# hkust-vgd/pointwise

Hardware: AMD Instinct MI355X
Metric: conv3p fwd+bwd Mpoints/s (higher is better)
Workload: dtype f32; 1 GPU; cfg2 ModelNet40-shaped: B=32 clouds/GPU x N=2048, pointcnn2_acsd conv3p stack 3->9 s1, 9->9 s2, 9->9 s3, 9->9 s4 (+SELU), forward+backward, a different batch every step, next batch's neighbour search enqueued on a side stream under the current backward; global_batch=32, points_per_cloud=2048, parallelism=dp1, backward_kernel_choice=hint from Conv3pStack.tune() at set-up: short lists

## Files before the change

### include/conv3p.h

```cpp
#ifndef CONV3P_H
#define CONV3P_H

#include <stddef.h>
#include <stdint.h>

#ifdef __cplusplus
extern "C" {
#endif

#define CONV3P_ABI_VERSION 5

#define CONV3P_OK 0
#define CONV3P_ERR_INVALID_ARGUMENT 1
#define CONV3P_ERR_WORKSPACE 2
#define CONV3P_ERR_UNSUPPORTED 3
#define CONV3P_ERR_LAUNCH 4
#define CONV3P_ERR_NO_DEVICE 5

#define CONV3P_PASS_FORWARD 0
#define CONV3P_PASS_BACKWARD 1
#define CONV3P_PASS_NEIGHBOR_COUNT 2

size_t conv3p_workspace_bytes(int pass, int elem_bytes, int B, int N, int Cin, int Cout, int fz,
                              int fy, int fx);
// ... 284 lines not shown
                        size_t workspace_bytes, void *stream);

size_t conv3p_seg_head_weighted_workspace_bytes(size_t rows, int num_class);
int conv3p_seg_weight_total_f32(const int32_t *labels, size_t rows, int num_class, const float *class_weight,
                                const float *point_weight, double *total, void *workspace, size_t workspace_bytes,
                                void *stream);
int conv3p_seg_weight_total_f64(const int32_t *labels, size_t rows, int num_class, const double *class_weight,
                                const double *point_weight, double *total, void *workspace, size_t workspace_bytes,
                                void *stream);
int conv3p_seg_head_weighted_f32(const float *act, const int32_t *labels, size_t rows, int num_class,
                                 const float *class_weight, const float *point_weight, double label_smoothing,
                                 float grad_scale, const double *denominator, float *grad_act, int32_t *pred,
                                 double *loss_sum, int64_t *counts, void *workspace, size_t workspace_bytes, void *stream);
int conv3p_seg_head_weighted_f64(const double *act, const int32_t *labels, size_t rows, int num_class,
                                 const double *class_weight, const double *point_weight, double label_smoothing,
                                 double grad_scale, const double *denominator, double *grad_act, int32_t *pred,
                                 double *loss_sum, int64_t *counts, void *workspace, size_t workspace_bytes, void *stream);
size_t conv3p_seg_confusion_workspace_bytes(size_t rows, int num_class);
int conv3p_seg_confusion(const int32_t *labels, const int32_t *pred, size_t rows, int num_class, int64_t *confusion,
                         void *workspace, size_t workspace_bytes, void *stream);

#define CONV3P_OPT_MAX_TENSORS 16
int conv3p_momentum_step_f32(int n_tensors, float *const *params, const float *const *grads, float *const *accums,
                             const size_t *numels, float lr, float momentum, void *stream);
int conv3p_momentum_step_f64(int n_tensors, double *const *params, const double *const *grads, double *const *accums,
                             const size_t *numels, double lr, double momentum, void *stream);
int conv3p_fc_backward_step_f32(const float *x, float *W, float *b, const float *y, const float *dy, int M, int K, int N,
                                int act, float *dx, float *accum_W, float *accum_b, float lr, float momentum,
                                void *workspace, size_t workspace_bytes, void *stream);

size_t conv3p_grad_norm_workspace_bytes(void);
int conv3p_grad_norm_f32(int n_tensors, const float *const *grads, const size_t *numels, double *stats, int accumulate,
                         void *workspace, size_t workspace_bytes, void *stream);
int conv3p_grad_norm_f64(int n_tensors, const double *const *grads, const size_t *numels, double *stats, int accumulate,
                         void *workspace, size_t workspace_bytes, void *stream);
int conv3p_momentum_step_guarded_f32(int n_tensors, float *const *params, const float *const *grads, float *const *accums,
                                     const size_t *numels, float lr, float momentum, int nesterov, float clip_norm,
                                     int skip_nonfinite, const double *stats, void *stream);
int conv3p_momentum_step_guarded_f64(int n_tensors, double *const *params, const double *const *grads,
                                     double *const *accums, const size_t *numels, double lr, double momentum, int nesterov,
                                     double clip_norm, int skip_nonfinite, const double *stats, void *stream);

size_t conv3p_cls_tail_workspace_bytes(int M, int H, int C);
int conv3p_cls_tail_f32(const float *fc1, const float *W2, const float *b2, const int32_t *labels, int M, int H, int C,
                        int training, double rate, const float *keep_mask, uint64_t seed, uint64_t step, float grad_scale,
                        float *logits, int32_t *pred, float *dfc1, float *dW2, float *db2, uint8_t *keep_out,
                        double *loss_sum, int64_t *counts, void *workspace, size_t workspace_bytes, void *stream);
int conv3p_cls_tail_step_f32(const float *fc1, float *W2, float *b2, const int32_t *labels, int M, int H, int C,
                             int training, double rate, const float *keep_mask, uint64_t seed, uint64_t step,
                             float grad_scale, float *logits, int32_t *pred, float *dfc1, float *accum_W2, float *accum_b2,
                             float lr, float momentum, uint8_t *keep_out, double *loss_sum, int64_t *counts,
                             void *workspace, size_t workspace_bytes, void *stream);

int conv3p_profile_enable(int on);
int conv3p_profile_reset(void);
int conv3p_profile_kinds(void);
const char *conv3p_profile_name(int kind);
int conv3p_profile_read(int kind, uint64_t *launches, double *total_ms);

const char *conv3p_status_string(int status);
int conv3p_abi_version(void);

#ifdef __cplusplus
}
#endif
#endif
```

### pointwise_amd/_lib.py

```python
import ctypes
import os

_HERE = os.path.dirname(os.path.abspath(__file__))
LIB_PATH = os.environ.get("CONV3P_HIP_LIB") or os.path.join(_HERE, "csrc", "libconv3p_hip.so")

OK = 0
ERR_INVALID_ARGUMENT = 1
ERR_WORKSPACE = 2
ERR_UNSUPPORTED = 3
ERR_LAUNCH = 4
ERR_NO_DEVICE = 5

PASS_FORWARD = 0
PASS_BACKWARD = 1
PASS_NEIGHBOR_COUNT = 2
CACHE_POINTS_UNCHANGED = 1
CACHE_SPARSE_NEIGHBOURHOODS = 2
CACHE_DENSE_NEIGHBOURHOODS = 8
CACHE_PREPARE_DEEP_ORDERS = 4
CACHE_FUSED_FORWARD = 16
CACHE_FUSED_BACKWARD = 32
CACHE_FUSED_STACK = CACHE_FUSED_FORWARD | CACHE_FUSED_BACKWARD
CACHE_MATMUL_BF16 = 64
ABI_VERSION = 5
# ... 93 lines not shown
                                       ctypes.c_double, ctypes.c_double, ctypes.c_uint64, ctypes.c_uint64, _vp, _vp, _vp,
                                       _vp, _vp, _vp, _vp, _vp, _vp, _vp, _sz, _vp]),
    "conv3p_sort_order_workspace_bytes": (_sz, [_i, _i, _i]),
    "conv3p_sort_order_f32": (_i, [_vp, _i, _i, _i, _i, _vp, _vp, _sz, _vp]),
    "conv3p_provider_wide_workspace_bytes": (_sz, [_i, _i, _i]),
    "conv3p_scene_blocks_workspace_bytes": (_sz, [ctypes.c_int64, _i, _i, ctypes.c_float, ctypes.c_float]),
    "conv3p_scene_blocks_f32": (_i, [_vp, _vp, ctypes.c_int64, _i, _i, ctypes.c_float, ctypes.c_float, _i, _i, _i,
                                     ctypes.c_uint64, ctypes.c_uint64, _vp, _vp, _vp, _vp, _vp, _vp, _vp, _sz, _vp]),
    "conv3p_scene_vote": (_i, [_vp, _vp, _sz, ctypes.c_int64, _i, _vp, _vp]),
    "conv3p_scene_vote_labels_workspace_bytes": (_sz, [ctypes.c_int64, _i]),
    "conv3p_scene_vote_labels": (_i, [_vp, ctypes.c_int64, _i, _vp, _vp, _vp, _sz, _vp]),
    "conv3p_scene_blocks_cover_workspace_bytes": (_sz, [ctypes.c_int64, _i, _i, ctypes.c_float, ctypes.c_float]),
    "conv3p_scene_blocks_cover_f32": (_i, [_vp, _vp, ctypes.c_int64, _i, _i, ctypes.c_float, ctypes.c_float, _i, _i, _i,
                                           ctypes.c_uint64, ctypes.c_uint64, _vp, _vp, _vp, _vp, _vp, _vp, _vp, _sz, _vp]),
    "conv3p_scene_blocks_rooms_workspace_bytes": (_sz, [ctypes.c_int64, ctypes.c_int64, _i, _i, ctypes.c_float,
                                                        ctypes.c_float, _i]),
    "conv3p_scene_blocks_rooms_f32": (_i, [_vp, _vp, _vp, ctypes.c_int64, ctypes.c_int64, _i, _i, ctypes.c_float,
                                           ctypes.c_float, _i, _i, _i, _i, ctypes.c_uint64, ctypes.c_uint64, _vp, _vp, _vp,
                                           _vp, _vp, _vp, _vp, _vp, _vp, _vp, _sz, _vp]),
    "conv3p_scene_vote_scores_f32": (_i, [_vp, _vp, _sz, ctypes.c_int64, _i, _vp, _vp, _vp]),
    "conv3p_scene_score_labels_workspace_bytes": (_sz, [ctypes.c_int64, _i]),
    "conv3p_scene_score_labels": (_i, [_vp, ctypes.c_int64, _i, _vp, _vp, _vp, _sz, _vp]),
    "conv3p_grid_subsample_workspace_bytes": (_sz, [ctypes.c_int64, _i]),
    "conv3p_grid_subsample_f32": (_i, [_vp, _vp, ctypes.c_int64, _i, _i, ctypes.c_float, _i, _i, _i, _vp, _vp, _vp, _vp, _vp,
                                       _vp, _vp, _vp, _sz, _vp]),
    "conv3p_grid_project_labels": (_i, [_vp, _vp, ctypes.c_int64, ctypes.c_int64, _vp, _vp]),
    "conv3p_grid_subsample_rooms_workspace_bytes": (_sz, [ctypes.c_int64, ctypes.c_int64, _i]),
    "conv3p_grid_subsample_rooms_f32": (_i, [_vp, _vp, _vp, ctypes.c_int64, ctypes.c_int64, _i, _i, ctypes.c_float, _i, _i, _i,
                                             _vp, _vp, _vp, _vp, _vp, _vp, _vp, _vp, _vp, _vp, _vp, _sz, _vp]),
    "conv3p_grid_neighbors": (_i, [_vp, _vp, _vp, _vp, _i, ctypes.c_int64, _vp, _vp]),
    "conv3p_grid_interpolate_f32": (_i, [_vp, ctypes.c_int64, _i, _vp, _vp, _i, _vp, _vp, ctypes.c_int64, _i, _vp, _i, _vp,
                                         _vp, _vp, _vp]),
    "conv3p_grid_interpolate_i64": (_i, [_vp, ctypes.c_int64, _i, _vp, _vp, _i, _vp, _vp, ctypes.c_int64, _i, _vp, _i, _vp,
                                         _vp, _vp, _vp]),
    "conv3p_grid_interpolate_rings_workspace_bytes": (_sz, [ctypes.c_int64]),
    "conv3p_grid_interpolate_rings_f32": (_i, [_vp, ctypes.c_int64, _i, _vp, _vp, _i, _vp, _vp, _vp, _vp, ctypes.c_int64, _vp,
                                               _vp, ctypes.c_int64, _i, _vp, _i, _i, _vp, _vp, _vp, _vp, _vp, _vp, _sz, _vp]),
    "conv3p_grid_interpolate_rings_i64": (_i, [_vp, ctypes.c_int64, _i, _vp, _vp, _i, _vp, _vp, _vp, _vp, ctypes.c_int64, _vp,
                                               _vp, ctypes.c_int64, _i, _vp, _i, _i, _vp, _vp, _vp, _vp, _vp, _vp, _sz, _vp]),
    "conv3p_grid_normals_f32": (_i, [_vp, _i, _vp, _vp, _vp, _vp, ctypes.c_int64, ctypes.c_int64, _i, _vp, _vp, _vp, _vp, _vp,
                                     _vp, _vp]),
    "conv3p_grid_segments_workspace_bytes": (_sz, [ctypes.c_int64]),
    "conv3p_grid_segments": (_i, [_vp, _vp, ctypes.c_int64, _vp, _vp, ctypes.c_int64, _i, _i, _vp, _vp, _vp, _vp, _vp, _vp, _vp,
                                  _sz, _vp]),
    "conv3p_grid_absorb_workspace_bytes": (_sz, [ctypes.c_int64]),
    "conv3p_grid_absorb_segments": (_i, [_vp, _vp, ctypes.c_int64, _vp, _vp, _vp, _vp, _vp, ctypes.c_int64, _i, _i, _i, _i, _vp,
                                         _vp, _vp, _vp, _sz, _vp]),
    "conv3p_stack_scratch_bytes": (_sz, [ctypes.POINTER(StackDesc), _i, _i, _i]),
    "conv3p_workspace_bytes": (_sz, [_i] * 9),
    "conv3p_cache_bytes": (_sz, [_i, _i, _i, ctypes.POINTER(CacheConfig)]),
    "conv3p_cache_forget": (_i, [_vp]),
    "conv3p_cache_init": (_i, [_vp, _sz, _vp]),
    "conv3p_cache_fused_status": (_i, [_vp, ctypes.POINTER(ctypes.c_uint), ctypes.POINTER(ctypes.c_uint), ctypes.POINTER(ctypes.c_uint)]),
    "conv3p_profile_enable": (_i, [_i]),
    "conv3p_profile_reset": (_i, []),
    "conv3p_profile_kinds": (_i, []),
    "conv3p_profile_name": (ctypes.c_char_p, [_i]),
    "conv3p_profile_read": (_i, [_i, ctypes.POINTER(ctypes.c_uint64), ctypes.POINTER(ctypes.c_double)]),
    "conv3p_status_string": (ctypes.c_char_p, [_i]),
    "conv3p_abi_version": (_i, []),
}
for _sfx, _real in (("f32", ctypes.c_float), ("f64", ctypes.c_double)):
    for _name, _s in _sig(_real).items():
        SYMBOLS["conv3p_%s_%s" % (_name, _sfx)] = _s

SYMBOLS["conv3p_provider_batch_wide_f32"] = SYMBOLS["conv3p_provider_batch_f32"]

_LIB = None


class Conv3pLibraryError(RuntimeError):
    pass


def load():
    global _LIB
    if _LIB is not None:
        return _LIB
    if not os.path.exists(LIB_PATH):
        raise Conv3pLibraryError(
            "libconv3p_hip.so not found at %s -- run `python -m pointwise_amd.build` "
            "(there is no CPU fallback in the product path)" % LIB_PATH)
    lib = ctypes.CDLL(LIB_PATH)
    for name, (res, args) in SYMBOLS.items():
        try:
            fn = getattr(lib, name)
        except AttributeError:
            raise Conv3pLibraryError("libconv3p_hip.so does not export %s" % name)
        fn.restype = res
        fn.argtypes = args
    if lib.conv3p_abi_version() != ABI_VERSION:
        raise Conv3pLibraryError("libconv3p_hip.so ABI version mismatch")
    _LIB = lib
    return lib


def status_string(code):
    return load().conv3p_status_string(code).decode()
```

### pointwise_amd/csrc/conv3p_abi.hip

```cpp
#include "../../include/conv3p.h"
#include "conv3p_kernels.hpp"
#include "conv3p_stack_fused.hpp"
#include "conv3p_prestep.hpp"
#include "conv3p_head.hpp"
#include "conv3p_seg_head.hpp"
#include "conv3p_seg_head_weighted.hpp"
#include "conv3p_optim.hpp"
#include "conv3p_optim_guarded.hpp"
#include "conv3p_cls_tail.hpp"
#include "conv3p_provider.hpp"
#include "conv3p_sort_wide.hpp"
#include "conv3p_scene.hpp"
#include "conv3p_scene_cover.hpp"
#include "conv3p_scene_rooms.hpp"
#include "conv3p_grid.hpp"
#include "conv3p_grid_rooms.hpp"
#include "conv3p_grid_interp.hpp"
#include "conv3p_grid_interp_rings.hpp"
#include "conv3p_grid_normals.hpp"
#include "conv3p_grid_segments.hpp"

#include <hip/hip_runtime.h>
#include <algorithm>
#include <cmath>
#include <cstdio>
#include <cstdlib>
#include <cstring>
#include <map>
#include <mutex>
#include <vector>

using namespace conv3p;

namespace {

constexpr size_t kAlign = 256;
inline size_t up(size_t x) { return (x + kAlign - 1) / kAlign * kAlign; }

enum Kind { K_PREP = 0, K_SEARCH, K_FORWARD, K_BACKWARD, K_REDUCE, K_SELU, K_SELU_GRAD, K_MEMSET,
            K_DEEP_GEMM, K_DEEP_DW, K_TRANSPOSE, K_DEEP_ORDER, K_FC_FWD, K_FC_DX, K_FC_DW, K_DEEP_GEMM_BF16, K_DEEP_DW_BF16,
            K_GENERIC_FWD, K_GENERIC_BWD,
            K_SEG_HEAD,
            K_NKINDS };
const char *const kKindName[K_NKINDS] = {"prep_kernel", "search_kernel", "forward_kernel",
                                         "backward_kernel", "reduce_partials_kernel", "selu_kernel",
                                         "selu_grad_kernel", "memset", "deep_gemm_kernel", "deep_dw_kernel",
                                         "transpose_filter_kernel", "deep_order_kernel", "fc_forward_kernel",
                                         "fc_dx_kernel", "fc_dw_kernel", "deep_gemm_bf16_kernel", "deep_dw_bf16_kernel",
                                         "generic_forward_kernel", "generic_backward_kernel", "seg_head_kernel"};
struct Prof {
    std::mutex mu;
    bool on = false;
    struct Rec { int kind; hipEvent_t a, b; };
    std::vector<Rec> recs;
    std::vector<hipEvent_t> pool;
    hipEvent_t get()
    {
        if (!pool.empty()) { hipEvent_t e = pool.back(); pool.pop_back(); return e; }
        hipEvent_t e = nullptr;
        (void)hipEventCreate(&e);
        return e;
    }
} g_prof;

struct Scope {
    hipStream_t s;
    hipEvent_t b = nullptr;
    bool on;
    Scope(int kind, hipStream_t stream) : s(stream)
    {
        std::lock_guard<std::mutex> lk(g_prof.mu);
        on = g_prof.on;
        if (!on) return;
        hipEvent_t a = g_prof.get();
        b = g_prof.get();
        (void)hipEventRecord(a, s);
// ... 359 lines not shown
    return hip_ok();
}

template <typename SlotT> inline const uint32_t *sched_of(const SlotT &S)
{
#ifdef CONV3P_DEV_NO_SCHED
    return nullptr;
#else
    return S.sched;
#endif
}

constexpr unsigned long long kShortListsPerPoint = 35, kShortListsPerPointFused = 48;
template <typename T> bool fused_ok(const Call<T> &c);
template <typename T> SchedJob make_sched_job(const Call<T> &c, int slot, bool fused)
{
    const auto &S = c.L.slot[slot];
    return SchedJob{S.segs, S.sched, S.cursor, S.regime,
                    (fused ? kShortListsPerPointFused : kShortListsPerPoint) * (unsigned long long)c.d.B * (unsigned long long)c.d.N};
}

#ifndef CONV3P_DEV_FUSED_M
#define CONV3P_DEV_FUSED_M 6
#endif
template <typename T> bool fused_ok(const Call<T> &c)
{
#ifdef CONV3P_DEV_NO_FUSED_SEARCH
    return false;
#endif
    const Stencil<T> &st = c.st;
    if (c.L.ftab == nullptr || st.window) return false;
    for (int a = 0; a < 3; ++a)
        if (st.ext[a] > kFMaxExt) return false;
    return true;
}
template <typename T> FusedJob<T> make_fused_job(const Call<T> &c)
{
    const auto &S = c.L.slot[c.slot];
    FusedJob<T> j;
    j.st = c.st;
    j.cc = c.cc;
    j.count = S.count;
    j.tcount = S.tcount;
    j.pairs = S.pairs;
    j.segs = S.segs;
    j.qsegs = S.qsegs;
    j.qbm = S.qbm;
    j.qbm_hi = S.qbm_hi;
    for (int a = 0; a < 3; ++a)
        for (int k = 0; k < kFMaxExt; ++k)
            j.clo[a][k] = (float)(((double)k * c.st.step[a] - (double)c.st.full[a] * 0.5) * (double)kFR);
    return j;
}
inline int fused_mask_depth(int elem, int ntiles, int ntap_max, int maxfull_max)
{
    const int mmax = (ntiles + kWavesPerBlock - 1) / kWavesPerBlock;
    int M = std::min(mmax, (int)CONV3P_DEV_FUSED_M);
    if (ntiles <= 32) M = 1;
    if (M < 1) M = 1;
    while (M > 1 && fused_lds(ntap_max, maxfull_max, elem, M).total > 40 * 1024) --M;
    return fused_lds(ntap_max, maxfull_max, elem, M).total > kMaxLds ? 0 : M;
}
template <typename T> int launch_fused(const Call<T> &c, const FusedJobs<T> &jobs, const SchedJobs &sjobs, int njobs, bool schedule = true)
{
    const Dims &d = c.d;
    const BlockMap bm = make_blockmap(d);
    int ntap_max = 1, maxfull_max = 1;
    for (int k = 0; k < njobs; ++k) {
        ntap_max = std::max(ntap_max, jobs.job[k].st.ntap);
        maxfull_max = std::max(maxfull_max, jobs.job[k].st.maxfull);
    }
    const int M = fused_mask_depth((int)sizeof(T), d.ntiles, ntap_max, maxfull_max);
    if (M == 0) return CONV3P_ERR_UNSUPPORTED;
#ifdef CONV3P_DEV_FUSED_LDS_KB
    const size_t lds = std::max(fused_lds(ntap_max, maxfull_max, (int)sizeof(T), M).total, (size_t)CONV3P_DEV_FUSED_LDS_KB * 1024);
#else
    const size_t lds = fused_lds(ntap_max, maxfull_max, (int)sizeof(T), M).total;
#endif
    if (lds > kMaxLds) return CONV3P_ERR_UNSUPPORTED;
    const float inv16 = (float)((double)kFR / (double)c.st.voxel);
    Scope sc(K_SEARCH, c.s);
    hipLaunchKernelGGL(tile_tables_kernel<T>, dim3((d.ntiles + kWavesPerBlock - 1) / kWavesPerBlock, d.B), dim3(256), 0, c.s,
                       c.L.pts, d.ntiles, inv16, c.L.ftab, c.cc.version, c.L.tab_version, c.L.tab_ticket, c.L.tab_inv, c.cc.force);
    bool ext3 = true;
    for (int k = 0; k < njobs; ++k)
        for (int a = 0; a < 3; ++a) ext3 &= jobs.job[k].st.ext[a] == 3;
    auto launch = [&](auto kern) {
        (void)hipFuncSetAttribute(reinterpret_cast<const void *>(kern), hipFuncAttributeMaxDynamicSharedMemorySize, (int)lds);
        hipLaunchKernelGGL(kern, dim3(grid_of(bm), njobs), dim3(256), lds, c.s, c.L.pts, c.L.boxes, c.L.ftab, d.N, d.ntiles,
                           c.L.ngroups, bm, jobs, M, inv16);
    };
    if (ext3) launch(search_fused_kernel<T, true>);
    else launch(search_fused_kernel<T, false>);
#ifndef CONV3P_DEV_NO_SCHED
    if (schedule)
        hipLaunchKernelGGL(tile_sched_kernel, dim3(8, njobs), dim3(1024), 0, c.s, sjobs, d.B, d.ntiles, c.L.ngroups, bm.rounds * d.ntiles);
#endif
    return hip_ok();
}

template <typename T> int add_companions(const Call<T> &c, FusedJobs<T> &fj, SchedJobs &sj, int n);
template <typename T> void note_companions_built(const Call<T> &c, const FusedJobs<T> &fj, int n);

template <typename T> int run_search(const Call<T> &c, int32_t *count, bool with_pairs)
{
    if (c.skip_search && with_pairs) return CONV3P_OK;
    const Dims &d = c.d;
    const Stencil<T> &st = c.st;
    const auto &S = c.L.slot[c.slot];
    if (fused_ok(c) && fused_mask_depth((int)sizeof(T), d.ntiles, st.ntap, st.maxfull) > 0 && (!with_pairs || count == S.count)) {
        FusedJobs<T> fj;
        SchedJobs sj;
        fj.job[0] = make_fused_job(c);
        sj.job[0] = make_sched_job(c, c.slot, true);
        if (!with_pairs) {
            FusedJob<T> &j = fj.job[0];
            j.count = count;
            j.tcount = nullptr;
            j.pairs = nullptr;
            j.segs = nullptr;
            j.qsegs = nullptr;
            j.qbm = nullptr;
            j.qbm_hi = nullptr;
            return launch_fused<T>(c, fj, sj, 1, false);
        }
        const int nj = add_companions<T>(c, fj, sj, 1);
        TRY(launch_fused<T>(c, fj, sj, nj));
        note_companions_built<T>(c, fj, nj);
        return CONV3P_OK;
    }
    const size_t lds = search_lds_bytes(st, c.L.gtiles);
    if (lds > kMaxLds) return CONV3P_ERR_UNSUPPORTED;
    const BlockMap bm = make_blockmap(d);
    {
        Scope sc(K_SEARCH, c.s);
        auto launch = [&](auto kern, const T *cmin) {
            (void)hipFuncSetAttribute(reinterpret_cast<const void *>(kern), hipFuncAttributeMaxDynamicSharedMemorySize, (int)lds);
            hipLaunchKernelGGL(kern, dim3(grid_of(bm)), dim3(256), lds, c.s, c.L.pts, c.L.boxes, st, d.N, d.ntiles,
                               c.L.gtiles, c.L.ngroups, bm, count, with_pairs ? S.pairs : nullptr, c.cc, S.segs, S.qsegs,
                               cmin, with_pairs ? S.tcount : nullptr, with_pairs ? S.qbm : nullptr, with_pairs ? S.qbm_hi : nullptr);
        };
        if (st.window) launch(search_kernel<T, true>, c.L.cmin);
        else launch(search_kernel<T, false>, static_cast<const T *>(nullptr));
        if (with_pairs) {
            SchedJobs sj;
            sj.job[0] = make_sched_job(c, c.slot, false);
// ... 3741 lines not shown
    if (dx != nullptr) {
        Scope sc(K_FC_DX, s);
        const int psteps = (N / 8 + 7) / 8 * 8;
        size_t lds = (size_t)32 * (8 * psteps + 4) * 4;
        const int nw = waves_for(lds <= 80 * 1024 ? 512 : 256);
        if (lds < (size_t)nw * 32 * 33 * 4) lds = (size_t)nw * 32 * 33 * 4;
        (void)hipFuncSetAttribute(reinterpret_cast<const void *>(fc_dx_kernel), hipFuncAttributeMaxDynamicSharedMemorySize, (int)lds);
        hipLaunchKernelGGL(fc_dx_kernel, dim3((unsigned)((K + 32 * nw - 1) / (32 * nw)), (unsigned)p.mblocks), dim3(64 * nw), lds, s, dz, W,
                           M, K, N, dx);
    }
    TRY(hip_ok());
    {
        Scope sc(K_FC_DW, s);
        auto launch = [&](auto kern, int steps) {
            const size_t lds = (size_t)2 * steps * (N + 1) * 4;
            const int nw = waves_for(lds <= 80 * 1024 ? 512 : 256);
            (void)hipFuncSetAttribute(reinterpret_cast<const void *>(kern), hipFuncAttributeMaxDynamicSharedMemorySize, (int)lds);
            hipLaunchKernelGGL(kern, dim3((unsigned)((K + 32 * nw - 1) / (32 * nw))), dim3(64 * nw), lds, s, x, dz, M, K, N, W,
                               accum_W, lr, momentum);
        };
        if (M <= 32) launch(fc_dw_step_kernel<16>, 16);
        else if (M <= 64) launch(fc_dw_step_kernel<32>, 32);
        else launch(fc_dw_step_kernel<64>, 64);
    }
    return hip_ok();
}

size_t conv3p_cls_tail_workspace_bytes(int M, int H, int C)
{
    ClsPlan p;
    return cls_plan(M, H, C, p) ? p.total : 0;
}
int conv3p_cls_tail_f32(const float *fc1, const float *W2, const float *b2, const int32_t *labels, int M, int H, int C,
                        int training, double rate, const float *keep_mask, uint64_t seed, uint64_t step, float grad_scale,
                        float *logits, int32_t *pred, float *dfc1, float *dW2, float *db2, uint8_t *keep_out,
                        double *loss_sum, int64_t *counts, void *workspace, size_t workspace_bytes, void *stream)
{
    return cls_tail_impl(fc1, const_cast<float *>(W2), const_cast<float *>(b2), labels, M, H, C, training, rate, keep_mask,
                         seed, step, grad_scale, logits, pred, dfc1, dW2, db2, nullptr, nullptr, 0.0f, 0.0f, keep_out,
                         loss_sum, counts, workspace, workspace_bytes, stream);
}
int conv3p_cls_tail_step_f32(const float *fc1, float *W2, float *b2, const int32_t *labels, int M, int H, int C,
                             int training, double rate, const float *keep_mask, uint64_t seed, uint64_t step,
                             float grad_scale, float *logits, int32_t *pred, float *dfc1, float *accum_W2, float *accum_b2,
                             float lr, float momentum, uint8_t *keep_out, double *loss_sum, int64_t *counts,
                             void *workspace, size_t workspace_bytes, void *stream)
{
    if (!accum_W2 || !accum_b2 || !dfc1) return CONV3P_ERR_INVALID_ARGUMENT;
    return cls_tail_impl(fc1, W2, b2, labels, M, H, C, training, rate, keep_mask, seed, step, grad_scale, logits, pred, dfc1,
                         nullptr, nullptr, accum_W2, accum_b2, lr, momentum, keep_out, loss_sum, counts, workspace,
                         workspace_bytes, stream);
}

int conv3p_profile_enable(int on)
{
    std::lock_guard<std::mutex> lk(g_prof.mu);
    g_prof.on = on != 0;
    return CONV3P_OK;
}
int conv3p_profile_reset(void)
{
    std::lock_guard<std::mutex> lk(g_prof.mu);
    for (auto &r : g_prof.recs) {
        g_prof.pool.push_back(r.a);
        g_prof.pool.push_back(r.b);
    }
    g_prof.recs.clear();
    return CONV3P_OK;
}
int conv3p_profile_kinds(void) { return K_NKINDS; }
const char *conv3p_profile_name(int kind) { return kind >= 0 && kind < K_NKINDS ? kKindName[kind] : ""; }
int conv3p_profile_read(int kind, uint64_t *launches, double *total_ms)
{
    std::lock_guard<std::mutex> lk(g_prof.mu);
    uint64_t n = 0;
    double ms = 0.0;
    for (auto &r : g_prof.recs) {
        if (r.kind != kind) continue;
        if (hipEventSynchronize(r.b) != hipSuccess) return CONV3P_ERR_LAUNCH;
        float t = 0.f;
        if (hipEventElapsedTime(&t, r.a, r.b) != hipSuccess) return CONV3P_ERR_LAUNCH;
        ms += t;
        ++n;
    }
    if (launches) *launches = n;
    if (total_ms) *total_ms = ms;
    return CONV3P_OK;
}

const char *conv3p_status_string(int status)
{
    switch (status) {
    case CONV3P_OK: return "ok";
    case CONV3P_ERR_INVALID_ARGUMENT: return "invalid argument";
    case CONV3P_ERR_WORKSPACE: return "workspace / cache null, misaligned or too small";
    case CONV3P_ERR_UNSUPPORTED: return "unsupported configuration";
    case CONV3P_ERR_LAUNCH: return "HIP launch error";
    case CONV3P_ERR_NO_DEVICE: return "no HIP device";
    default: return "unknown status";
    }
}
int conv3p_abi_version(void) { return CONV3P_ABI_VERSION; }

}
```

### pointwise_amd/csrc/conv3p_search_fused.hpp

```cpp
#pragma once

#include "conv3p_device.hpp"

namespace conv3p {

constexpr int kFR = 16;
constexpr int kFK = 96;
constexpr int kFEntries = 116;
constexpr int kFHeader = 3 * kFEntries;
constexpr int kFTableU64 = kFHeader + 4;
constexpr int kFMaxExt = 8;
#ifndef CONV3P_DEV_FUSED_ABLATE
#define CONV3P_DEV_FUSED_ABLATE 0
#endif
constexpr int kFStream = 192;
constexpr int kFMaxE = 12;

__device__ __forceinline__ int floor_i32(float x)
{
    int r;
    asm("v_cvt_flr_i32_f32_e32 %0, %1" : "=v"(r) : "v"(x));
    return r;
}
__device__ __forceinline__ bool finite3(float x, float y, float z)
// ... 180 lines not shown
    const T vv[3] = {v.x, v.y, v.z};
    fwd = kNoTap;
    bwd = kNoTap;
    bool exact = in;
    if (TapFast<T>::enabled) {
        int t[3];
        bool near = false;
#pragma unroll
        for (int a = 0; a < 3; ++a) {
            const float q = (float)d[a] * (float)rvoxel;
            const float mag = fmaxf(fabsf((float)c.p[a]), fabsf((float)vv[a]));
            near |= fabsf(q - __builtin_rintf(q)) <= __builtin_fmaf(mag, 5.0e-7f * (float)rvoxel, 1.0e-6f * (float)st.full[a]);
            t[a] = (int)q;
        }
        exact = in && near;
        if (in && !near) {
            const int tx = tapmap[clamp_tap(t[0], st.full[0])];
            const int ty = tapmap[st.maxfull + clamp_tap(t[1], st.full[1])];
            const int tz = tapmap[2 * st.maxfull + clamp_tap(t[2], st.full[2])];
            if ((tx | ty | tz) >= 0) {
                fwd = (uint32_t)((tz * st.ext[1] + ty) * st.ext[0] + tx);
                bwd = (uint32_t)st.ntap - 1u - fwd;
            }
        }
    }
    if (exact) {
        const int tx = tapmap[clamp_tap((int)(d[0] / st.voxel), st.full[0])];
        const int ty = tapmap[st.maxfull + clamp_tap((int)(d[1] / st.voxel), st.full[1])];
        const int tz = tapmap[2 * st.maxfull + clamp_tap((int)(d[2] / st.voxel), st.full[2])];
        if ((tx | ty | tz) >= 0) {
            fwd = (uint32_t)((tz * st.ext[1] + ty) * st.ext[0] + tx);
            if (want_bwd) {
                const T lx = (T)((double)v.x - st.half[0]), ly = (T)((double)v.y - st.half[1]), lz = (T)((double)v.z - st.half[2]);
                const int bx = tapmap[clamp_tap((int)((c.p[0] - lx) / st.voxel), st.full[0])];
                const int by = tapmap[st.maxfull + clamp_tap((int)((c.p[1] - ly) / st.voxel), st.full[1])];
                const int bz = tapmap[2 * st.maxfull + clamp_tap((int)((c.p[2] - lz) / st.voxel), st.full[2])];
                if ((bx | by | bz) >= 0) bwd = (uint32_t)((bz * st.ext[1] + by) * st.ext[0] + bx);
            }
        }
    }
    if (fwd != kNoTap) {
        atomicAdd(&cnt[fwd * kCntStride + ql], 1u);
        if (want_bm && bwd != kNoTap) atomicOr(&bmk[ql + ((bwd >> 5) << 6)], 1u << (bwd & 31u));
    }
}

typedef int int4_a4 __attribute__((ext_vector_type(4), aligned(4)));

template <typename T> __device__ __forceinline__ bool fused_compacts(const Stencil<T> &st, uint32_t tile_hits)
{
    return !(CONV3P_DEV_FUSED_ABLATE & 16) && (st.step[0] * st.step[1] * st.step[2] > 1 || tile_hits > 48u * 64u);
}

template <typename T, bool EXT3>
__global__ __launch_bounds__(256) void search_fused_kernel(const PointRec<T> *__restrict__ pts, const T *__restrict__ boxes,
                                                           const unsigned long long *__restrict__ tables, int N, int ntiles,
                                                           int ngroups, BlockMap bm, FusedJobs<T> jobs, int M, float inv16)
{
    extern __shared__ __attribute__((aligned(16))) char smem[];
    const int wave = threadIdx.x >> 6, lane = threadIdx.x & 63;
    int b, qt;
    if (!block_to_cloud(bm, b, qt)) return;
    const FusedJob<T> &job = jobs.job[blockIdx.y];
    const bool have_pairs = job.pairs != nullptr;
    if (have_pairs && slot_valid(job.cc, b)) return;
    const Stencil<T> &st = job.st;

    const FusedLds L = fused_lds(st.ntap, st.maxfull, (int)sizeof(T), M);
    int16_t *tapmap = reinterpret_cast<int16_t *>(smem + L.tapmap);
    uint32_t *cnt = reinterpret_cast<uint32_t *>(smem + L.cnt);
    CenRec<T> *cen = reinterpret_cast<CenRec<T> *>(smem + L.cen);
    uint32_t *bmk = reinterpret_cast<uint32_t *>(smem + L.bmk);
    uint32_t *nqw = reinterpret_cast<uint32_t *>(smem + L.nqw);
    uint32_t *misc = reinterpret_cast<uint32_t *>(smem + L.misc);
    T *red = reinterpret_cast<T *>(smem + L.red);
    unsigned long long *tab = reinterpret_cast<unsigned long long *>(smem + L.tab) + (size_t)wave * kFTableU64;
    unsigned long long *masks = reinterpret_cast<unsigned long long *>(smem + L.masks) + (size_t)wave * M * 64;

    const PointRec<T> *cloud_pts = pts + (size_t)b * ntiles * kTile;
    const T *cloud_box = boxes + (size_t)b * ntiles * 6;
    const unsigned long long *cloud_tab = tables + (size_t)b * ntiles * kFTableU64;
    const PointRec<T> me = cloud_pts[(size_t)qt * kTile + lane];
    const float pf[3] = {(float)me.x, (float)me.y, (float)me.z};
    const bool qvalid = me.idx >= 0 && finite3(pf[0], pf[1], pf[2]);
    const bool want_bm = job.qbm != nullptr && (st.ntap <= 32 || (st.ntap <= 128 && job.qbm_hi != nullptr));

    build_tapmap(tapmap, st.full, st.step, st.maxfull);
    for (int e = threadIdx.x; e < st.ntap * kCntStride; e += blockDim.x) cnt[e] = 0;
    if (wave == 0) {
        CenRec<T> r;
        const T p[3] = {me.x, me.y, me.z};
#pragma unroll
        for (int a = 0; a < 3; ++a) {
            r.lo[a] = (T)((double)p[a] - st.half[a]);
            r.hi[a] = (T)((double)p[a] + st.half[a]);
            r.p[a] = p[a];
            r.pad[a] = (T)0;
        }
        cen[lane] = r;
        bmk[lane] = 0;
        if (st.ntap > 32) bmk[64 + lane] = 0;
        if (st.ntap > 64) bmk[128 + lane] = bmk[192 + lane] = 0;
    } else {
        const int a = wave - 1;
        const T pa = a == 0 ? me.x : (a == 1 ? me.y : me.z);
        const T mn = wave_min(qvalid ? pa : Limits<T>::inf()), mx = wave_max(qvalid ? pa : -Limits<T>::inf());
        if (lane == 0) {
            red[a] = mn;
            red[3 + a] = mx;
        }
    }
    const float q0[3] = {1.0e-3f + 4.0e-6f * (fabsf(pf[0]) * inv16), 1.0e-3f + 4.0e-6f * (fabsf(pf[1]) * inv16),
                         1.0e-3f + 4.0e-6f * (fabsf(pf[2]) * inv16)};
    __syncthreads();
    T ulo[3], uhi[3];
#pragma unroll
    for (int a = 0; a < 3; ++a) {
        ulo[a] = (T)((double)red[a] - st.half[a]);
        uhi[a] = (T)((double)red[3 + a] + st.half[a]);
    }
    const float s16[3] = {(float)(kFR * st.step[0]), (float)(kFR * st.step[1]), (float)(kFR * st.step[2])};

    auto for_my_tiles = [&](auto &&visit) {
        for (int base = 0; base < ntiles; base += 64) {
            uint64_t todo = tiles_meeting(cloud_box, ntiles, base, ulo, uhi) & (0x1111111111111111ull << wave);
            while (todo) {
                const int i = __builtin_ctzll(todo);
                todo &= todo - 1;
                visit(base + i, todo ? base + __builtin_ctzll(todo) : -1);
            }
        }
    };
    uint4 pf0 = make_uint4(0, 0, 0, 0), pf1 = pf0, pf2 = pf0;
    int pf_ct = -1;
    auto request = [&](int ct) {
        const uint4 *src = reinterpret_cast<const uint4 *>(cloud_tab + (size_t)ct * kFTableU64);
        pf0 = src[lane];
        pf1 = src[64 + lane];
        pf2 = src[128 + (lane < kFTableU64 / 2 - 128 ? lane : 0)];
        pf_ct = ct;
    };
    auto compute_mask = [&](int ct, int nxt) -> uint64_t {
        if (pf_ct != ct) request(ct);
        uint4 *dst = reinterpret_cast<uint4 *>(tab);
        __builtin_amdgcn_wave_barrier();
        dst[lane] = pf0;
        dst[64 + lane] = pf1;
        if (lane < kFTableU64 / 2 - 128) dst[128 + lane] = pf2;
        __builtin_amdgcn_wave_barrier();
        if (nxt >= 0) request(nxt);
        if (CONV3P_DEV_FUSED_ABLATE & 4) return 0ull;
        const uint64_t h0 = tab[kFHeader], h1 = tab[kFHeader + 1];
        const float tmin[3] = {__builtin_bit_cast(float, (uint32_t)h0), __builtin_bit_cast(float, (uint32_t)(h0 >> 32)),
                               __builtin_bit_cast(float, (uint32_t)h1)};
        const int e = (int)(uint32_t)(h1 >> 32);
        const int es = e > kFMaxE ? kFMaxE : e;
        const int ws = (kFR >> es) + 2;
        float gs[3], smax = 0.0f;
#pragma unroll
        for (int a = 0; a < 3; ++a) {
            const float g = (pf[a] - tmin[a]) * inv16;
            const float slack = __builtin_fmaf(4.0e-6f, fabsf(g), q0[a]);
            smax = fmaxf(smax, slack);
            gs[a] = (g - slack) + (float)(ws << es);
        }
        const bool wide = e > kFMaxE || __any(qvalid && !(smax <= 0.2f * (float)(1 << es)));
        auto entry = [&](float x) {
            int j = floor_i32(x) >> es;
            return j < 0 ? 0 : (j > kFEntries - 1 ? kFEntries - 1 : j);
        };
        uint64_t h;
        if (wide) {
            h = tab[kFHeader + 2];
        } else if (EXT3) {
            uint64_t A[3];
#pragma unroll
            for (int a = 0; a < 3; ++a) {
                const float x1 = gs[a] - (float)(kFR / 2);
                const unsigned long long *ta = tab + a * kFEntries;
                const uint64_t r0 = ta[entry(x1 - s16[a])], r1 = ta[entry(x1)], r2 = ta[entry(x1 + s16[a])];
                A[a] = r0 | r1 | r2;
            }
            h = A[0] & A[1] & A[2];
        } else {
            h = fused_mask(job, tab, gs, es);
        }
        return qvalid ? h : 0ull;
    };

    {
        uint32_t mine = 0;
        int ord = 0;
        for_my_tiles([&](int ct, int nxt) {
            const uint64_t m = compute_mask(ct, nxt);
            mine += (uint32_t)__popcll(m);
            if (ord < M) masks[(size_t)ord * 64 + lane] = m;
            ++ord;
        });
        nqw[wave * 64 + lane] = mine;
    }
    __syncthreads();

    if (wave == 0) {
        const uint32_t n0 = nqw[lane], n1 = nqw[64 + lane], n2 = nqw[128 + lane], n3 = nqw[192 + lane];
        const uint32_t nq = n0 + n1 + n2 + n3;
        int Ltot;
        const uint32_t offq = (uint32_t)wave_excl_scan((int)nq, Ltot);
        const uint32_t cap = job.cc.pairs_per_cloud;
        uint32_t base = 0, ok = 0;
        if (!have_pairs) {
            if (lane == 0) misc[0] = misc[1] = misc[2] = 0;
        } else {
        if (lane == 0) {
            base = Ltot ? atomicAdd(&job.cc.cursor[b], (uint32_t)Ltot) : 0u;
            ok = (base <= cap && (uint32_t)Ltot <= cap - base) ? 1u : 0u;
            if (!ok) atomicSub(&job.cc.cursor[b], (uint32_t)Ltot);
            base += (uint32_t)b * cap;
            job.segs[((size_t)b * ntiles + qt) * ngroups] = ok ? make_uint2(base, (uint32_t)Ltot) : make_uint2(0u, kSegOverflow);
            for (int g = 1; g < ngroups; ++g) job.segs[((size_t)b * ntiles + qt) * ngroups + g] = make_uint2(0u, 0u);
            misc[0] = base;
            misc[1] = ok;
            misc[2] = (uint32_t)Ltot;
        }
        base = __shfl(base, 0);
        ok = __shfl(ok, 0);
        if (!ok || !fused_compacts(st, (uint32_t)Ltot))
            job.qsegs[((size_t)b * ntiles + qt) * ngroups * 64 + lane] = ok ? make_uint2(base + offq, nq) : make_uint2(0u, kSegOverflow);
        for (int g = 1; g < ngroups; ++g) job.qsegs[(((size_t)b * ntiles + qt) * ngroups + g) * 64 + lane] = make_uint2(0u, 0u);
        }
        nqw[lane] = offq;
        nqw[64 + lane] = offq + n0;
        nqw[128 + lane] = offq + n0 + n1;
        nqw[192 + lane] = offq + n0 + n1 + n2;
    }
    __syncthreads();
    const bool ok = misc[1] != 0;
    const uint32_t gbase = misc[0];
    char *pbase = reinterpret_cast<char *>(job.pairs + gbase);
    const T rvoxel = (T)1 / st.voxel;

    if (!(CONV3P_DEV_FUSED_ABLATE & 2)) {
        uint32_t *sdesc = reinterpret_cast<uint32_t *>(smem + L.stream) + wave * (2 * kFStream);
        uint32_t *sslot = sdesc + kFStream;
        uint32_t off = nqw[wave * 64 + lane] * 8u;
        int have = 0, ord = 0;
        pf_ct = -1;
        auto drain = [&](int n) {
            if (CONV3P_DEV_FUSED_ABLATE & 1) return;
            constexpr int kU = 2;
            uint32_t d[kU], so[kU];
            PointRec<T> v[kU];
#pragma unroll
            for (int u = 0; u < kU; ++u) {
                const int i = u * 64 + lane;
                d[u] = sdesc[i < n ? i : 0];
                so[u] = sslot[i < n ? i : 0];
            }
#pragma unroll
            for (int u = 0; u < kU; ++u) v[u] = cloud_pts[(size_t)((d[u] >> 12) * kTile + (d[u] & 63u))];
#pragma unroll
            for (int u = 0; u < kU; ++u) {
                const bool on = u * 64 + lane < n;
                const uint32_t ql = (d[u] >> 6) & 63u;
                uint32_t fwd, bwd;
                fused_resolve<T>(st, rvoxel, tapmap, cnt, bmk, cen, ql, v[u], on, true, want_bm, fwd, bwd);
                if (on && ok) {
                    PairEntry pe;
                    pe.cand = (uint32_t)v[u].idx;
                    pe.code = pair_code(fwd, bwd, ql);
                    *reinterpret_cast<PairEntry *>(pbase + so[u]) = pe;
                }
            }
        };
        for_my_tiles([&](int ct, int nxt) {
            uint64_t mm = ord < M ? masks[(size_t)ord * 64 + lane] : compute_mask(ct, nxt);
            ++ord;
            const uint32_t dbase = ((uint32_t)ct << 12) | ((uint32_t)lane << 6);
            while (true) {
                const uint64_t act = __ballot(mm != 0);
                if (act == 0) break;
                if (mm != 0) {
                    const uint32_t c = (uint32_t)__builtin_ctzll(mm);
                    mm &= mm - 1;
                    const int at = have + (int)__builtin_amdgcn_mbcnt_hi((uint32_t)(act >> 32), __builtin_amdgcn_mbcnt_lo((uint32_t)act, 0));
                    sdesc[at] = dbase | c;
                    sslot[at] = off;
                    off += 8u;
                }
                have += __popcll(act);
                __builtin_amdgcn_wave_barrier();
                if (have >= 128) {
                    drain(128);
                    __builtin_amdgcn_wave_barrier();
                    const uint32_t cd = sdesc[128 + lane], cs = sslot[128 + lane];
                    __builtin_amdgcn_wave_barrier();
                    sdesc[lane] = cd;
                    sslot[lane] = cs;
                    have -= 128;
                    __builtin_amdgcn_wave_barrier();
                }
            }
        });
        if (have > 0) drain(have);
    }
    __threadfence_block();
    __syncthreads();

    if (have_pairs && ok && fused_compacts(st, misc[2])) {
        uint32_t *livec = nqw + 64;
        {
            const int c = wave * 16 + (lane & 15);
            uint32_t sacc = 0;
            for (int f = lane >> 4; f < st.ntap; f += 4) sacc += cnt[f * kCntStride + c];
            sacc += lane_xor16(sacc);
            sacc += lane_xor32(sacc);
            if (lane < 16) livec[c] = sacc;
        }
        __builtin_amdgcn_wave_barrier();
        const uint32_t r0 = nqw[wave * 16], r1 = wave == kWavesPerBlock - 1 ? misc[2] : nqw[wave * 16 + 16];
        PairEntry *tp = job.pairs + gbase;
        const uint64_t lt = lane == 0 ? 0ull : (~0ull >> (64 - lane));
        uint32_t carry = 0;
        constexpr int kCB = 4;
        PairEntry cur[kCB], nxt[kCB];
        auto request = [&](PairEntry (&dst)[kCB], uint32_t pos) {
#pragma unroll
            for (int u = 0; u < kCB; ++u) {
                const uint32_t i = pos + (uint32_t)(u * 64 + lane);
                dst[u] = tp[i < r1 ? i : r0];
            }
        };
        if (r0 < r1) request(nxt, r0);
        for (uint32_t pos = r0; pos < r1; pos += 64 * kCB) {
#pragma unroll
            for (int u = 0; u < kCB; ++u) cur[u] = nxt[u];
            if (pos + 64 * kCB < r1) request(nxt, pos + 64 * kCB);
#pragma unroll
            for (int u = 0; u < kCB; ++u) {
                const uint32_t cpos = pos + (uint32_t)(u * 64);
                if (cpos >= r1) break;
                const uint32_t i = cpos + (uint32_t)lane;
                const bool valid = i < r1;
                const uint32_t c = code_q(cur[u].code) & 63u;
                const bool live = valid && code_fwd(cur[u].code) != kNoTap;
                const uint32_t oc = nqw[c], lv = livec[c];
                const uint64_t Lm = __ballot(live);
                const uint32_t sc = oc > cpos ? oc - cpos : 0u;
                const uint64_t before = Lm & lt & ~((1ull << (sc & 63u)) - 1ull);
                const uint32_t rank = (uint32_t)__popcll(before) + (oc < cpos ? carry : 0u);
                if (live && oc + rank != i) tp[oc + rank] = cur[u];
                if (valid && i - oc >= lv) {
                    PairEntry dead;
                    dead.cand = cur[u].cand;
                    dead.code = pair_code(kNoTap, kNoTap, c);
                    tp[i] = dead;
// ... 54 lines not shown
```

Baseline: 167.0 Mpoints/s.

## Keep first tile masks in registers and pop them as a window

Result: no change. 168.6 Mpoints/s, median of 6 (+1.0%).

```diff
diff --git a/include/conv3p.h b/include/conv3p.h
--- a/include/conv3p.h
+++ b/include/conv3p.h
@@ -360,6 +360,8 @@
                              float lr, float momentum, uint8_t *keep_out, double *loss_sum, int64_t *counts,
                              void *workspace, size_t workspace_bytes, void *stream);
 
+int conv3p_dev_search_window(int on);
+
 int conv3p_profile_enable(int on);
 int conv3p_profile_reset(void);
 int conv3p_profile_kinds(void);
diff --git a/pointwise_amd/_lib.py b/pointwise_amd/_lib.py
--- a/pointwise_amd/_lib.py
+++ b/pointwise_amd/_lib.py
@@ -169,6 +169,7 @@
     "conv3p_cache_forget": (_i, [_vp]),
     "conv3p_cache_init": (_i, [_vp, _sz, _vp]),
     "conv3p_cache_fused_status": (_i, [_vp, ctypes.POINTER(ctypes.c_uint), ctypes.POINTER(ctypes.c_uint), ctypes.POINTER(ctypes.c_uint)]),
+    "conv3p_dev_search_window": (_i, [_i]),
     "conv3p_profile_enable": (_i, [_i]),
     "conv3p_profile_reset": (_i, []),
     "conv3p_profile_kinds": (_i, []),
diff --git a/pointwise_amd/csrc/conv3p_abi.hip b/pointwise_amd/csrc/conv3p_abi.hip
--- a/pointwise_amd/csrc/conv3p_abi.hip
+++ b/pointwise_amd/csrc/conv3p_abi.hip
@@ -22,6 +22,7 @@
 
 #include <hip/hip_runtime.h>
 #include <algorithm>
+#include <atomic>
 #include <cmath>
 #include <cstdio>
 #include <cstdlib>
@@ -487,6 +488,7 @@
             j.clo[a][k] = (float)(((double)k * c.st.step[a] - (double)c.st.full[a] * 0.5) * (double)kFR);
     return j;
 }
+static std::atomic<bool> g_search_window{true};
 inline int fused_mask_depth(int elem, int ntiles, int ntap_max, int maxfull_max)
 {
     const int mmax = (ntiles + kWavesPerBlock - 1) / kWavesPerBlock;
@@ -525,8 +527,11 @@
         hipLaunchKernelGGL(kern, dim3(grid_of(bm), njobs), dim3(256), lds, c.s, c.L.pts, c.L.boxes, c.L.ftab, d.N, d.ntiles,
                            c.L.ngroups, bm, jobs, M, inv16);
     };
-    if (ext3) launch(search_fused_kernel<T, true>);
-    else launch(search_fused_kernel<T, false>);
+    const bool window = g_search_window.load(std::memory_order_relaxed);
+    if (ext3 && window) launch(search_fused_kernel<T, true, kFWindow>);
+    else if (ext3) launch(search_fused_kernel<T, true, 0>);
+    else if (window) launch(search_fused_kernel<T, false, kFWindow>);
+    else launch(search_fused_kernel<T, false, 0>);
 #ifndef CONV3P_DEV_NO_SCHED
     if (schedule)
         hipLaunchKernelGGL(tile_sched_kernel, dim3(8, njobs), dim3(1024), 0, c.s, sjobs, d.B, d.ntiles, c.L.ngroups, bm.rounds * d.ntiles);
@@ -4374,6 +4379,12 @@
                          workspace_bytes, stream);
 }
 
+int conv3p_dev_search_window(int on)
+{
+    const bool was = g_search_window.exchange(on != 0, std::memory_order_relaxed);
+    return was ? 1 : 0;
+}
+
 int conv3p_profile_enable(int on)
 {
     std::lock_guard<std::mutex> lk(g_prof.mu);
diff --git a/pointwise_amd/csrc/conv3p_search_fused.hpp b/pointwise_amd/csrc/conv3p_search_fused.hpp
--- a/pointwise_amd/csrc/conv3p_search_fused.hpp
+++ b/pointwise_amd/csrc/conv3p_search_fused.hpp
@@ -256,13 +256,18 @@
     return !(CONV3P_DEV_FUSED_ABLATE & 16) && (st.step[0] * st.step[1] * st.step[2] > 1 || tile_hits > 48u * 64u);
 }
 
-template <typename T, bool EXT3>
-__global__ __launch_bounds__(256) void search_fused_kernel(const PointRec<T> *__restrict__ pts, const T *__restrict__ boxes,
+#ifndef CONV3P_DEV_FUSED_KWIN
+#define CONV3P_DEV_FUSED_KWIN 4
+#endif
+constexpr int kFWindow = CONV3P_DEV_FUSED_KWIN;
+template <typename T, bool EXT3, int KWIN>
+__global__ __launch_bounds__(256, sizeof(T) == 4 ? 5 : 4)
+    void search_fused_kernel(const PointRec<T> *__restrict__ pts, const T *__restrict__ boxes,
                                                            const unsigned long long *__restrict__ tables, int N, int ntiles,
                                                            int ngroups, BlockMap bm, FusedJobs<T> jobs, int M, float inv16)
 {
     extern __shared__ __attribute__((aligned(16))) char smem[];
-    const int wave = threadIdx.x >> 6, lane = threadIdx.x & 63;
+    const int wave = __builtin_amdgcn_readfirstlane(threadIdx.x >> 6), lane = threadIdx.x & 63;
     int b, qt;
     if (!block_to_cloud(bm, b, qt)) return;
     const FusedJob<T> &job = jobs.job[blockIdx.y];
@@ -325,7 +330,7 @@
     }
     const float s16[3] = {(float)(kFR * st.step[0]), (float)(kFR * st.step[1]), (float)(kFR * st.step[2])};
 
-    auto for_my_tiles = [&](auto &&visit) {
+    auto for_my_tiles = [&](auto &&visit) __attribute__((always_inline)) {
         for (int base = 0; base < ntiles; base += 64) {
             uint64_t todo = tiles_meeting(cloud_box, ntiles, base, ulo, uhi) & (0x1111111111111111ull << wave);
             while (todo) {
@@ -337,14 +342,14 @@
     };
     uint4 pf0 = make_uint4(0, 0, 0, 0), pf1 = pf0, pf2 = pf0;
     int pf_ct = -1;
-    auto request = [&](int ct) {
+    auto request = [&](int ct) __attribute__((always_inline)) {
         const uint4 *src = reinterpret_cast<const uint4 *>(cloud_tab + (size_t)ct * kFTableU64);
         pf0 = src[lane];
         pf1 = src[64 + lane];
         pf2 = src[128 + (lane < kFTableU64 / 2 - 128 ? lane : 0)];
         pf_ct = ct;
     };
-    auto compute_mask = [&](int ct, int nxt) -> uint64_t {
+    auto compute_mask = [&](int ct, int nxt) __attribute__((always_inline)) -> uint64_t {
         if (pf_ct != ct) request(ct);
         uint4 *dst = reinterpret_cast<uint4 *>(tab);
         __builtin_amdgcn_wave_barrier();
@@ -392,15 +397,32 @@
         return qvalid ? h : 0ull;
     };
 
+    static_assert(KWIN >= 0 && KWIN <= 4, "the window's slots are four named variables");
+    uint64_t w0 = 0, w1 = 0, w2 = 0, w3 = 0;
+    int t0 = 0, t1 = 0, t2 = 0, t3 = 0;
+    auto put = [&](int sl, uint64_t m, int ct) __attribute__((always_inline)) {
+        const uint64_t a0 = w0, a1 = w1, a2 = w2, a3 = w3;
+        const int b0 = t0, b1 = t1, b2 = t2, b3 = t3;
+        w0 = sl == 0 ? m : a0, t0 = sl == 0 ? ct : b0;
+        if (KWIN > 1) w1 = sl == 1 ? m : a1, t1 = sl == 1 ? ct : b1;
+        if (KWIN > 2) w2 = sl == 2 ? m : a2, t2 = sl == 2 ? ct : b2;
+        if (KWIN > 3) w3 = sl == 3 ? m : a3, t3 = sl == 3 ? ct : b3;
+    };
+    int ntl = 0;
     {
         uint32_t mine = 0;
         int ord = 0;
-        for_my_tiles([&](int ct, int nxt) {
+        for_my_tiles([&](int ct, int nxt) __attribute__((always_inline)) {
             const uint64_t m = compute_mask(ct, nxt);
             mine += (uint32_t)__popcll(m);
-            if (ord < M) masks[(size_t)ord * 64 + lane] = m;
+            if (ord < KWIN) {
+                put(ord, m, ct);
+            } else if (ord - KWIN < M) {
+                masks[(size_t)(ord - KWIN) * 64 + lane] = m;
+            }
             ++ord;
         });
+        ntl = ord;
         nqw[wave * 64 + lane] = mine;
     }
     __syncthreads();
@@ -449,7 +471,7 @@
         uint32_t off = nqw[wave * 64 + lane] * 8u;
         int have = 0, ord = 0;
         pf_ct = -1;
-        auto drain = [&](int n) {
+        auto drain = [&](int n) __attribute__((always_inline)) {
             if (CONV3P_DEV_FUSED_ABLATE & 1) return;
             constexpr int kU = 2;
             uint32_t d[kU], so[kU];
@@ -476,35 +498,81 @@
                 }
             }
         };
-        for_my_tiles([&](int ct, int nxt) {
-            uint64_t mm = ord < M ? masks[(size_t)ord * 64 + lane] : compute_mask(ct, nxt);
-            ++ord;
-            const uint32_t dbase = ((uint32_t)ct << 12) | ((uint32_t)lane << 6);
-            while (true) {
-                const uint64_t act = __ballot(mm != 0);
-                if (act == 0) break;
-                if (mm != 0) {
-                    const uint32_t c = (uint32_t)__builtin_ctzll(mm);
-                    mm &= mm - 1;
-                    const int at = have + (int)__builtin_amdgcn_mbcnt_hi((uint32_t)(act >> 32), __builtin_amdgcn_mbcnt_lo((uint32_t)act, 0));
-                    sdesc[at] = dbase | c;
-                    sslot[at] = off;
-                    off += 8u;
+        auto pop_round = [&](uint64_t act, uint64_t &mm, uint32_t tile12) __attribute__((always_inline)) {
+            if (mm != 0) {
+                const uint32_t c = (uint32_t)__builtin_ctzll(mm);
+                mm &= mm - 1;
+                const int at = have + (int)__builtin_amdgcn_mbcnt_hi((uint32_t)(act >> 32), __builtin_amdgcn_mbcnt_lo((uint32_t)act, 0));
+                sdesc[at] = tile12 | ((uint32_t)lane << 6) | c;
+                sslot[at] = off;
+                off += 8u;
+            }
+            have += __popcll(act);
+            __builtin_amdgcn_wave_barrier();
+            if (have >= 128) {
+                drain(128);
+                __builtin_amdgcn_wave_barrier();
+                const uint32_t cd = sdesc[128 + lane], cs = sslot[128 + lane];
+                __builtin_amdgcn_wave_barrier();
+                sdesc[lane] = cd;
+                sslot[lane] = cs;
+                have -= 128;
+                __builtin_amdgcn_wave_barrier();
+            }
+        };
+        if constexpr (KWIN == 0) {
+            for_my_tiles([&](int ct, int nxt) __attribute__((always_inline)) {
+                uint64_t mm = ord < M ? masks[(size_t)ord * 64 + lane] : compute_mask(ct, nxt);
+                ++ord;
+                while (true) {
+                    const uint64_t act = __ballot(mm != 0);
+                    if (act == 0) break;
+                    pop_round(act, mm, (uint32_t)ct << 12);
                 }
-                have += __popcll(act);
-                __builtin_amdgcn_wave_barrier();
-                if (have >= 128) {
-                    drain(128);
-                    __builtin_amdgcn_wave_barrier();
-                    const uint32_t cd = sdesc[128 + lane], cs = sslot[128 + lane];
-                    __builtin_amdgcn_wave_barrier();
-                    sdesc[lane] = cd;
-                    sslot[lane] = cs;
-                    have -= 128;
-                    __builtin_amdgcn_wave_barrier();
+            });
+        } else {
+            auto pop_window = [&](int nw) __attribute__((always_inline)) {
+#ifdef CONV3P_DEV_FUSED_POP_BY_TILE
+                for (int k = 0; k < nw; ++k) {
+                    const uint64_t a0 = w0, a1 = w1, a2 = w2, a3 = w3;
+                    const int b0 = t0, b1 = t1, b2 = t2, b3 = t3;
+                    uint64_t mm = k == 0 ? a0 : k == 1 ? a1 : k == 2 ? a2 : a3;
+                    const uint32_t tile12 = (uint32_t)(k == 0 ? b0 : k == 1 ? b1 : k == 2 ? b2 : b3) << 12;
+                    while (true) {
+                        const uint64_t act = __ballot(mm != 0);
+                        if (act == 0) break;
+                        pop_round(act, mm, tile12);
+                    }
                 }
-            }
-        });
+#else
+                const uint64_t a1 = w1, a2 = w2, a3 = w3;
+                const uint32_t b1 = (uint32_t)t1 << 12, b2 = (uint32_t)t2 << 12, b3 = (uint32_t)t3 << 12;
+                uint64_t mm = w0;
+                uint32_t tile12 = (uint32_t)t0 << 12;
+                uint32_t ne = (nw > 1 && a1 != 0 ? 1u : 0u) | (nw > 2 && a2 != 0 ? 2u : 0u) | (nw > 3 && a3 != 0 ? 4u : 0u);
+                while (true) {
+                    if (mm == 0 && ne != 0) {
+                        const uint32_t s = (uint32_t)__builtin_ctz(ne);
+                        ne &= ne - 1;
+                        mm = s == 0 ? a1 : s == 1 ? a2 : a3;
+                        tile12 = s == 0 ? b1 : s == 1 ? b2 : b3;
+                    }
+                    const uint64_t act = __ballot(mm != 0);
+                    if (act == 0) break;
+                    pop_round(act, mm, tile12);
+                }
+#endif
+            };
+            if (ntl > 0) pop_window(ntl < KWIN ? ntl : KWIN);
+            if (ntl > KWIN)
+                for_my_tiles([&](int ct, int nxt) __attribute__((always_inline)) {
+                    const int o = ord++;
+                    if (o < KWIN) return;
+                    const int sl = o % KWIN;
+                    put(sl, o - KWIN < M ? masks[(size_t)(o - KWIN) * 64 + lane] : compute_mask(ct, nxt), ct);
+                    if (sl == KWIN - 1 || o == ntl - 1) pop_window(sl + 1);
+                });
+        }
         if (have > 0) drain(have);
     }
     __threadfence_block();
```
